# ArthurBrussee/brush

Measured on NVIDIA H100. Metric: fwd+bwd Mpix/s @1M Gaussians 1080p, higher is better.
Workload: dtype f32

## Files before the change

### brush_b200/csrc/bg_common.cuh

```cuda
#pragma once
#include <cuda_runtime.h>
#include <stdint.h>

#include "../../include/brush_b200.h"

namespace bg {

constexpr uint32_t TILE_W = 16;
constexpr uint32_t TILE_PIX = 256;
constexpr float ALPHA_CUTOFF_MID = 1.0f / 255.0f;
constexpr float ALPHA_CUTOFF_BAND = 1.0e-3f;

enum CtlOffsets : uint32_t {
    CTL_COUNTERS = 0,
    CTL_TICKETS = 16,
    CTL_HIST_DEPTH = 64,
    CTL_HIST_TILE = 64 + 1024,
    CTL_WORDS = 64 + 2048
};
enum TicketIds : uint32_t {
    TK_PROJECT = 0, TK_DEPTH_HIST = 1, TK_DEPTH_PASS0 = 2 , TK_SCAN = 6, TK_VISIBLE = 7,
    TK_TILE_HIST = 8, TK_TILE_PASS0 = 9 , TK_MISC = 13
};

constexpr uint32_t LB_INVALID = 0, LB_AGGREGATE = 1, LB_INCLUSIVE = 2;

__device__ __forceinline__ void lb_store(unsigned long long *p, uint32_t epoch, uint32_t status, uint32_t value) {
    unsigned long long w = ((unsigned long long)((epoch << 2) | status) << 32) | (unsigned long long)value;
    asm volatile("st.relaxed.gpu.global.u64 [%0], %1;" ::"l"(p), "l"(w) : "memory");
}
__device__ __forceinline__ unsigned long long lb_load(const unsigned long long *p) {
    unsigned long long w;
    asm volatile("ld.relaxed.gpu.global.u64 %0, [%1];" : "=l"(w) : "l"(p) : "memory");
    return w;
}
__device__ __forceinline__ uint32_t lb_status(unsigned long long w, uint32_t epoch) {
    uint32_t hi = (uint32_t)(w >> 32);
    return ((hi >> 2) == epoch) ? (hi & 3u) : LB_INVALID;
}
__device__ __forceinline__ uint32_t lb_value(unsigned long long w) { return (uint32_t)w; }

__device__ __forceinline__ uint32_t lb_lookback_warp(const unsigned long long *state, uint32_t tile, uint32_t epoch) {
    const uint32_t lane = threadIdx.x & 31u;
    uint32_t prefix = 0;
    int64_t pos = (int64_t)tile - 1;
    while (pos >= 0) {
        int64_t idx = pos - (int64_t)lane;
        uint32_t st, val;
        while (true) {
            st = LB_INCLUSIVE;
            val = 0;
            if (idx >= 0) {
                unsigned long long w = lb_load(state + idx);
                st = lb_status(w, epoch);
                val = lb_value(w);
            }
            if (__all_sync(0xffffffffu, st != LB_INVALID)) break;
        }
        uint32_t incl_mask = __ballot_sync(0xffffffffu, st == LB_INCLUSIVE);
        uint32_t first = incl_mask ? (uint32_t)(__ffs(incl_mask) - 1) : 32u;
        uint32_t contrib = (lane <= first) ? val : 0u;
        for (int o = 16; o > 0; o >>= 1) contrib += __shfl_xor_sync(0xffffffffu, contrib, o);
        prefix += contrib;
        if (incl_mask) break;
        pos -= 32;
    }
    return prefix;
}

__device__ __forceinline__ uint32_t smem_u32(const void *p) { return (uint32_t)__cvta_generic_to_shared(p); }
__device__ __forceinline__ void mbar_init(unsigned long long *bar, uint32_t count) {
    asm volatile("mbarrier.init.shared::cta.b64 [%0], %1;" ::"r"(smem_u32(bar)), "r"(count) : "memory");
    asm volatile("fence.mbarrier_init.release.cluster;" ::: "memory");
}
__device__ __forceinline__ void mbar_expect_tx(unsigned long long *bar, uint32_t bytes) {
    asm volatile("mbarrier.arrive.expect_tx.shared::cta.b64 _, [%0], %1;" ::"r"(smem_u32(bar)), "r"(bytes) : "memory");
}
__device__ __forceinline__ void tma_bulk_g2s(void *dst_smem, const void *src_gmem, uint32_t bytes, unsigned long long *bar) {
    asm volatile("cp.async.bulk.shared::cluster.global.mbarrier::complete_tx::bytes [%0], [%1], %2, [%3];" ::"r"(
                     smem_u32(dst_smem)),
                 "l"(src_gmem), "r"(bytes), "r"(smem_u32(bar))
                 : "memory");
}
__device__ __forceinline__ void mbar_wait(unsigned long long *bar, uint32_t parity) {
    asm volatile(
        "{\n"
        ".reg .pred p;\n"
        "WAIT_LOOP:\n"
        "mbarrier.try_wait.parity.shared::cta.b64 p, [%0], %1;\n"
        "@p bra WAIT_DONE;\n"
        "bra WAIT_LOOP;\n"
        "WAIT_DONE:\n"
        "}\n" ::"r"(smem_u32(bar)),
        "r"(parity)
        : "memory");
}

__device__ __forceinline__ float2 fadd2_rn(float2 a, float2 b) { return make_float2(__fadd_rn(a.x, b.x), __fadd_rn(a.y, b.y)); }
__device__ __forceinline__ float2 fmul2_rn(float2 a, float2 b) { return make_float2(__fmul_rn(a.x, b.x), __fmul_rn(a.y, b.y)); }
__device__ __forceinline__ float2 ffma2_rn(float2 a, float2 b, float2 c) {
    return make_float2(__fmaf_rn(a.x, b.x, c.x), __fmaf_rn(a.y, b.y, c.y));
}

__device__ __forceinline__ uint32_t block_exclusive_scan(uint32_t v, uint32_t *warp_sums, uint32_t *total) {
    const uint32_t lane = threadIdx.x & 31u, wid = threadIdx.x >> 5, nw = blockDim.x >> 5;
    uint32_t incl = v;
    for (int o = 1; o < 32; o <<= 1) {
        uint32_t t = __shfl_up_sync(0xffffffffu, incl, o);
        if (lane >= (uint32_t)o) incl += t;
    }
    if (lane == 31) warp_sums[wid] = incl;
    __syncthreads();
    if (wid == 0) {
        uint32_t s = (lane < nw) ? warp_sums[lane] : 0u;
        uint32_t si = s;
        for (int o = 1; o < 32; o <<= 1) {
            uint32_t t = __shfl_up_sync(0xffffffffu, si, o);
            if (lane >= (uint32_t)o) si += t;
        }
        if (lane < nw) warp_sums[lane] = si - s;
        if (lane == 31) warp_sums[32] = si;
    }
    __syncthreads();
    uint32_t r = warp_sums[wid] + incl - v;
    *total = warp_sums[32];
    __syncthreads();
    return r;
}

}
```

### brush_b200/csrc/blend_fwd.cu

```cuda
#include "blend_common.cuh"

namespace bg {

template <bool BWD_INFO, bool SMOOTH, bool DEPTH>
__global__ void __launch_bounds__(RASTER_THREADS)
blend_fwd_kernel(const float *__restrict__ projected, const uint32_t *__restrict__ cgid_from_isect,
                 uint32_t *__restrict__ tile_offsets, const uint32_t *__restrict__ gid_from_cgid,
                 float4 *__restrict__ out_f32, uint32_t *__restrict__ out_packed, float *__restrict__ visible,
                 uint32_t *__restrict__ live_masks, uint32_t *__restrict__ warp_batches, BlendUniforms u,
                 const float *__restrict__ depths, float *__restrict__ out_depth) {
    __shared__ BlendStage s_stage[RASTER_WARPS];
    __shared__ uint32_t s_max_useful;

    const uint32_t tile = blockIdx.x;
    const uint32_t tid = threadIdx.x, lane = tid & 31u, wid = tid >> 5;
    const uint32_t tile_x0 = (tile % u.tiles_x) * TILE_W, tile_y0 = (tile / u.tiles_x) * TILE_W;
    const uint32_t blk_x0 = tile_x0 + 8u * (wid & 1u), blk_y0 = tile_y0 + 8u * (wid >> 1);
    const uint32_t pix_x = blk_x0 + (lane & 7u), pix_y0 = blk_y0 + (lane >> 3), pix_y1 = pix_y0 + 4u;
    const bool inside0 = pix_x < u.img_w && pix_y0 < u.img_h;
    const bool inside1 = pix_x < u.img_w && pix_y1 < u.img_h;
    const float px = (float)pix_x + 0.5f, py0 = (float)pix_y0 + 0.5f;
    const float2 npy2 = make_float2(-py0, -(py0 + 4.0f));
    const float rx0 = (float)blk_x0 + 0.5f, rx1 = rx0 + 7.0f, ry0 = (float)blk_y0 + 0.5f, ry1 = ry0 + 7.0f;

    const uint32_t range_lo = tile_offsets[tile * 2], range_hi = tile_offsets[tile * 2 + 1];
    if (BWD_INFO && tid == 0) s_max_useful = range_lo;
    BlendStage &st = s_stage[wid];
    if (lane == 0) { mbar_init(&st.bar[0], 1); mbar_init(&st.bar[1], 1); }
    __syncthreads();
    uint32_t phase_bits = 0u;

    float2 T2 = make_float2(1.0f, 1.0f);
    float2 Tt2 = make_float2(inside0 ? 1.0f : 0.0f, inside1 ? 1.0f : 0.0f);
    float2 r2 = make_float2(0.0f, 0.0f), g2 = r2, b2 = r2, d2 = r2;
    uint32_t last_useful = range_lo;

    const uint32_t num_batches = (range_hi - range_lo + WB - 1) / WB;
    const size_t mbase = blend_mask_base(range_lo, tile) + wid;
    uint32_t batches_walked = 0;
    uint32_t next_id = 0;
    float next_z = 0.0f;
    auto prefetch = [&](uint32_t b) {
        const uint32_t start = range_lo + b * WB;
        const uint32_t count = min((uint32_t)WB, range_hi - start);
        const uint32_t id = lane < count ? __ldg(cgid_from_isect + start + lane) : 0u;
        next_id = id;
        if constexpr (DEPTH) next_z = lane < count ? __ldg(depths + id) : 0.0f;
        if (lane < count) st.ids[b & 1u][lane] = id;
        stage_rows_tma(st, b & 1u, count, projected, lane);
    };
    if (num_batches > 0 && __any_sync(0xffffffffu, inside0 || inside1)) {
        prefetch(0);
        for (uint32_t b = 0; b < num_batches; b++) {
            const uint32_t batch_start = range_lo + b * WB;
            const uint32_t count = min((uint32_t)WB, range_hi - batch_start);
            const uint32_t my_id = next_id;
            const float my_z = next_z;
            if (b + 1 < num_batches) prefetch(b + 1);
            mbar_wait(&st.bar[b & 1u], (phase_bits >> (b & 1u)) & 1u);
            phase_bits ^= 1u << (b & 1u);
            float *rows = st.rows[b & 1u];
            bool hit = false;
            if (lane < count) {
                float *mine = rows + lane * ROW;
                const float4 A = *reinterpret_cast<const float4 *>(mine);
                const float4 B = *reinterpret_cast<const float4 *>(mine + 4);
                const float bcol = mine[8];
                float pt = mine[ROW_PT];
                if constexpr (SMOOTH) pt += SMOOTH_THR_EXTRA;
                hit = block_may_hit(A.x, A.y, A.z, A.w, B.x, pt, rx0, rx1, ry0, ry1);
                *reinterpret_cast<float2 *>(mine + 6) = make_float2(fmaxf(B.z, 0.0f), fmaxf(B.w, 0.0f));
                mine[8] = fmaxf(bcol, 0.0f);
                if constexpr (DEPTH) mine[ROW_Z] = my_z;
            }
            uint32_t bits = __ballot_sync(0xffffffffu, hit);
            uint32_t used_m = 0, acted_m = 0;
            while (bits) {
                const uint32_t s = (uint32_t)__ffs(bits) - 1u;
                bits &= bits - 1u;
                const float *row = rows + s * ROW;
                const float4 A = *reinterpret_cast<const float4 *>(row);
                const float4 B = *reinterpret_cast<const float4 *>(row + 4);
                const float4 C = *reinterpret_cast<const float4 *>(row + 8);
                float2 dy2;
                const float2 sg = pair_sigma(A.x - px, A.y, C.y, C.z, C.w, npy2, dy2);
                const float2 gs = make_float2(ex2_approx(-sg.x), ex2_approx(-sg.y));
                const float2 oa = fmul2_rn(gs, bcast2(B.y));
                float a0 = fminf(0.999f, oa.x), a1 = fminf(0.999f, oa.y);
                bool act0, act1;
                if constexpr (SMOOTH) {
                    const float2 ae = smooth_alpha(make_float2(a0, a1), sg, act0, act1);
                    a0 = ae.x; a1 = ae.y;
                } else {
                    act0 = sg.x >= 0.0f && oa.x >= ALPHA_CUTOFF_MID; act1 = sg.y >= 0.0f && oa.y >= ALPHA_CUTOFF_MID;
                }
                const float2 nT = fmul2_rn(Tt2, fadd2_rn(make_float2(-a0, -a1), bcast2(1.0f)));
                const bool c0 = act0 && nT.x > 1.0e-4f, c1 = act1 && nT.y > 1.0e-4f;
                const float2 vis = fmul2_rn(make_float2(c0 ? a0 : 0.0f, c1 ? a1 : 0.0f), T2);
                r2 = ffma2_rn(bcast2(B.z), vis, r2);
                g2 = ffma2_rn(bcast2(B.w), vis, g2);
                b2 = ffma2_rn(bcast2(C.x), vis, b2);
                if constexpr (DEPTH) d2 = ffma2_rn(bcast2(row[ROW_Z]), vis, d2);
                const uint32_t bit = 1u << s;
                const bool acted = (Tt2.x > 1.0e-4f && act0) || (Tt2.y > 1.0e-4f && act1);
                if (c0 || c1) used_m |= bit;
                if (BWD_INFO && acted) acted_m |= bit;
                T2.x = c0 ? nT.x : T2.x;
                T2.y = c1 ? nT.y : T2.y;
                Tt2.x = act0 ? nT.x : Tt2.x;
                Tt2.y = act1 ? nT.y : Tt2.y;
            }
            const uint32_t used = __reduce_or_sync(0xffffffffu, used_m);
            if (BWD_INFO) {
                const uint32_t acted = __reduce_or_sync(0xffffffffu, acted_m);
                if (lane == 0) live_masks[mbase + (size_t)b * RASTER_WARPS] = acted;
                if ((used >> lane) & 1u) {
                    visible[__ldg(gid_from_cgid + my_id)] = 1.0f;
                    last_useful = batch_start + lane + 1;
                }
            }
            batches_walked = b + 1;
            if (__all_sync(0xffffffffu, !(Tt2.x > 1.0e-4f) && !(Tt2.y > 1.0e-4f))) {
                if (b + 1 < num_batches) mbar_wait(&st.bar[(b + 1) & 1u], (phase_bits >> ((b + 1) & 1u)) & 1u);
                break;
            }
            __syncwarp();
        }
    }

    auto write_pixel = [&](float T, float r, float g, float bl, float d, uint32_t pix_y) {
        const float fr = r + T * u.bg_r, fg = g + T * u.bg_g, fb = bl + T * u.bg_b, fa = 1.0f - T;
        const size_t pix_id = (size_t)pix_x + (size_t)pix_y * u.img_w;
        if (BWD_INFO) {
            out_f32[pix_id] = make_float4(fr, fg, fb, fa);
            if constexpr (DEPTH) out_depth[pix_id] = d;
        } else {
            uint32_t r8 = (uint32_t)fminf(fmaxf(fr * 255.0f, 0.0f), 255.0f);
            uint32_t g8 = (uint32_t)fminf(fmaxf(fg * 255.0f, 0.0f), 255.0f);
            uint32_t b8 = (uint32_t)fminf(fmaxf(fb * 255.0f, 0.0f), 255.0f);
            uint32_t a8 = (uint32_t)fminf(fmaxf(fa * 255.0f, 0.0f), 255.0f);
            out_packed[pix_id] = r8 | (g8 << 8) | (b8 << 16) | (a8 << 24);
        }
    };
    if (inside0) write_pixel(T2.x, r2.x, g2.x, b2.x, d2.x, pix_y0);
    if (inside1) write_pixel(T2.y, r2.y, g2.y, b2.y, d2.y, pix_y1);
    if (BWD_INFO) {
        if (lane == 0) warp_batches[tile * RASTER_WARPS + wid] = batches_walked;
        uint32_t m = last_useful;
        for (int o = 16; o > 0; o >>= 1) m = max(m, __shfl_xor_sync(0xffffffffu, m, o));
        __syncthreads();
        if (lane == 0 && m > range_lo) atomicMax(&s_max_useful, m);
        __syncthreads();
        if (tid == 0) tile_offsets[tile * 2 + 1] = s_max_useful;
    }
}

cudaError_t launch_blend_fwd(cudaStream_t s, bool bwd_info, bool smooth, uint32_t num_tiles, const float *projected,
                             const uint32_t *cgid_from_isect, uint32_t *tile_offsets, const uint32_t *gid_from_cgid, void *out_img,
                             float *visible, uint32_t *live_masks, uint32_t *warp_batches, uint32_t tiles_x, uint32_t w,
                             uint32_t h, const float *bg, const float *depths, float *out_depth) {
    BlendUniforms u;
    u.tiles_x = tiles_x; u.img_w = w; u.img_h = h; u.bg_r = bg[0]; u.bg_g = bg[1]; u.bg_b = bg[2];
#define BG_LAUNCH_FWD(B, S, D, F32, PACKED, LM, WBAT)                                                                    \
    blend_fwd_kernel<B, S, D><<<num_tiles, RASTER_THREADS, 0, s>>>(projected, cgid_from_isect, tile_offsets, gid_from_cgid, \
                                                                   F32, PACKED, visible, LM, WBAT, u, depths, out_depth)
    if (!bwd_info)
        BG_LAUNCH_FWD(false, false, false, nullptr, (uint32_t *)out_img, nullptr, nullptr);
    else if (out_depth && !smooth)
        BG_LAUNCH_FWD(true, false, true, (float4 *)out_img, nullptr, live_masks, warp_batches);
    else if (out_depth)
        BG_LAUNCH_FWD(true, true, true, (float4 *)out_img, nullptr, live_masks, warp_batches);
    else if (!smooth)
        BG_LAUNCH_FWD(true, false, false, (float4 *)out_img, nullptr, live_masks, warp_batches);
    else
        BG_LAUNCH_FWD(true, true, false, (float4 *)out_img, nullptr, live_masks, warp_batches);
#undef BG_LAUNCH_FWD
    return cudaGetLastError();
}

}
```

Before: 987.2.

## Use producer warp with shared 4-slot TMA ring for forward blend

New measurement: 1012 (median of 6 runs). 2.5% higher.

```diff
diff --git a/brush_b200/csrc/bg_common.cuh b/brush_b200/csrc/bg_common.cuh
--- a/brush_b200/csrc/bg_common.cuh
+++ b/brush_b200/csrc/bg_common.cuh
@@ -76,6 +76,9 @@
 __device__ __forceinline__ void mbar_expect_tx(unsigned long long *bar, uint32_t bytes) {
     asm volatile("mbarrier.arrive.expect_tx.shared::cta.b64 _, [%0], %1;" ::"r"(smem_u32(bar)), "r"(bytes) : "memory");
 }
+__device__ __forceinline__ void mbar_arrive(unsigned long long *bar) {
+    asm volatile("mbarrier.arrive.shared::cta.b64 _, [%0];" ::"r"(smem_u32(bar)) : "memory");
+}
 __device__ __forceinline__ void tma_bulk_g2s(void *dst_smem, const void *src_gmem, uint32_t bytes, unsigned long long *bar) {
     asm volatile("cp.async.bulk.shared::cluster.global.mbarrier::complete_tx::bytes [%0], [%1], %2, [%3];" ::"r"(
                      smem_u32(dst_smem)),
diff --git a/brush_b200/csrc/blend_fwd.cu b/brush_b200/csrc/blend_fwd.cu
--- a/brush_b200/csrc/blend_fwd.cu
+++ b/brush_b200/csrc/blend_fwd.cu
@@ -2,154 +2,178 @@
 
 namespace bg {
 
+constexpr int FWD_SLOTS = 4;
+constexpr int FWD_THREADS = RASTER_THREADS + 32;
+
+struct __align__(128) FwdSlot {
+    float rows[WB * ROW];
+    uint32_t ids[WB];
+    float z[WB];
+    uint32_t count;
+    unsigned long long full, empty;
+};
+
 template <bool BWD_INFO, bool SMOOTH, bool DEPTH>
-__global__ void __launch_bounds__(RASTER_THREADS)
+__global__ void __launch_bounds__(FWD_THREADS, 1)
 blend_fwd_kernel(const float *__restrict__ projected, const uint32_t *__restrict__ cgid_from_isect,
                  uint32_t *__restrict__ tile_offsets, const uint32_t *__restrict__ gid_from_cgid,
                  float4 *__restrict__ out_f32, uint32_t *__restrict__ out_packed, float *__restrict__ visible,
                  uint32_t *__restrict__ live_masks, uint32_t *__restrict__ warp_batches, BlendUniforms u,
                  const float *__restrict__ depths, float *__restrict__ out_depth) {
-    __shared__ BlendStage s_stage[RASTER_WARPS];
-    __shared__ uint32_t s_max_useful;
+    __shared__ FwdSlot s_slot[FWD_SLOTS];
+    __shared__ uint32_t s_max_useful, s_done;
 
     const uint32_t tile = blockIdx.x;
     const uint32_t tid = threadIdx.x, lane = tid & 31u, wid = tid >> 5;
-    const uint32_t tile_x0 = (tile % u.tiles_x) * TILE_W, tile_y0 = (tile / u.tiles_x) * TILE_W;
-    const uint32_t blk_x0 = tile_x0 + 8u * (wid & 1u), blk_y0 = tile_y0 + 8u * (wid >> 1);
-    const uint32_t pix_x = blk_x0 + (lane & 7u), pix_y0 = blk_y0 + (lane >> 3), pix_y1 = pix_y0 + 4u;
-    const bool inside0 = pix_x < u.img_w && pix_y0 < u.img_h;
-    const bool inside1 = pix_x < u.img_w && pix_y1 < u.img_h;
-    const float px = (float)pix_x + 0.5f, py0 = (float)pix_y0 + 0.5f;
-    const float2 npy2 = make_float2(-py0, -(py0 + 4.0f));
-    const float rx0 = (float)blk_x0 + 0.5f, rx1 = rx0 + 7.0f, ry0 = (float)blk_y0 + 0.5f, ry1 = ry0 + 7.0f;
-
     const uint32_t range_lo = tile_offsets[tile * 2], range_hi = tile_offsets[tile * 2 + 1];
-    if (BWD_INFO && tid == 0) s_max_useful = range_lo;
-    BlendStage &st = s_stage[wid];
-    if (lane == 0) { mbar_init(&st.bar[0], 1); mbar_init(&st.bar[1], 1); }
+    const uint32_t num_batches = (range_hi - range_lo + WB - 1) / WB;
+    if (tid == 0) { s_max_useful = range_lo; s_done = 0u; }
+    if (tid < FWD_SLOTS) { mbar_init(&s_slot[tid].full, 1); mbar_init(&s_slot[tid].empty, RASTER_WARPS); }
     __syncthreads();
-    uint32_t phase_bits = 0u;
-
-    float2 T2 = make_float2(1.0f, 1.0f);
-    float2 Tt2 = make_float2(inside0 ? 1.0f : 0.0f, inside1 ? 1.0f : 0.0f);
-    float2 r2 = make_float2(0.0f, 0.0f), g2 = r2, b2 = r2, d2 = r2;
-    uint32_t last_useful = range_lo;
-
-    const uint32_t num_batches = (range_hi - range_lo + WB - 1) / WB;
-    const size_t mbase = blend_mask_base(range_lo, tile) + wid;
-    uint32_t batches_walked = 0;
-    uint32_t next_id = 0;
-    float next_z = 0.0f;
-    auto prefetch = [&](uint32_t b) {
-        const uint32_t start = range_lo + b * WB;
-        const uint32_t count = min((uint32_t)WB, range_hi - start);
-        const uint32_t id = lane < count ? __ldg(cgid_from_isect + start + lane) : 0u;
-        next_id = id;
-        if constexpr (DEPTH) next_z = lane < count ? __ldg(depths + id) : 0.0f;
-        if (lane < count) st.ids[b & 1u][lane] = id;
-        stage_rows_tma(st, b & 1u, count, projected, lane);
-    };
-    if (num_batches > 0 && __any_sync(0xffffffffu, inside0 || inside1)) {
-        prefetch(0);
-        for (uint32_t b = 0; b < num_batches; b++) {
-            const uint32_t batch_start = range_lo + b * WB;
-            const uint32_t count = min((uint32_t)WB, range_hi - batch_start);
-            const uint32_t my_id = next_id;
-            const float my_z = next_z;
-            if (b + 1 < num_batches) prefetch(b + 1);
-            mbar_wait(&st.bar[b & 1u], (phase_bits >> (b & 1u)) & 1u);
-            phase_bits ^= 1u << (b & 1u);
-            float *rows = st.rows[b & 1u];
-            bool hit = false;
+
+    if (wid == RASTER_WARPS) {
+        auto load_ids = [&](uint32_t b) {
+            const uint32_t start = range_lo + b * WB;
+            return lane < min((uint32_t)WB, range_hi - start) ? __ldg(cgid_from_isect + start + lane) : 0u;
+        };
+        uint32_t b = 0;
+        uint32_t next_id = num_batches > 0 ? load_ids(0) : 0u;
+        for (; b < num_batches; b++) {
+            if (*reinterpret_cast<volatile uint32_t *>(&s_done) == (uint32_t)RASTER_WARPS) break;
+            const uint32_t id = next_id;
+            if (b + 1 < num_batches) next_id = load_ids(b + 1);
+            FwdSlot &sl = s_slot[b % FWD_SLOTS];
+            if (b >= FWD_SLOTS) mbar_wait(&sl.empty, ((b / FWD_SLOTS) & 1u) ^ 1u);
+            const uint32_t count = min((uint32_t)WB, range_hi - (range_lo + b * WB));
             if (lane < count) {
-                float *mine = rows + lane * ROW;
-                const float4 A = *reinterpret_cast<const float4 *>(mine);
-                const float4 B = *reinterpret_cast<const float4 *>(mine + 4);
-                const float bcol = mine[8];
-                float pt = mine[ROW_PT];
-                if constexpr (SMOOTH) pt += SMOOTH_THR_EXTRA;
-                hit = block_may_hit(A.x, A.y, A.z, A.w, B.x, pt, rx0, rx1, ry0, ry1);
-                *reinterpret_cast<float2 *>(mine + 6) = make_float2(fmaxf(B.z, 0.0f), fmaxf(B.w, 0.0f));
-                mine[8] = fmaxf(bcol, 0.0f);
-                if constexpr (DEPTH) mine[ROW_Z] = my_z;
-            }
-            uint32_t bits = __ballot_sync(0xffffffffu, hit);
-            uint32_t used_m = 0, acted_m = 0;
-            while (bits) {
-                const uint32_t s = (uint32_t)__ffs(bits) - 1u;
-                bits &= bits - 1u;
-                const float *row = rows + s * ROW;
-                const float4 A = *reinterpret_cast<const float4 *>(row);
-                const float4 B = *reinterpret_cast<const float4 *>(row + 4);
-                const float4 C = *reinterpret_cast<const float4 *>(row + 8);
-                float2 dy2;
-                const float2 sg = pair_sigma(A.x - px, A.y, C.y, C.z, C.w, npy2, dy2);
-                const float2 gs = make_float2(ex2_approx(-sg.x), ex2_approx(-sg.y));
-                const float2 oa = fmul2_rn(gs, bcast2(B.y));
-                float a0 = fminf(0.999f, oa.x), a1 = fminf(0.999f, oa.y);
-                bool act0, act1;
-                if constexpr (SMOOTH) {
-                    const float2 ae = smooth_alpha(make_float2(a0, a1), sg, act0, act1);
-                    a0 = ae.x; a1 = ae.y;
-                } else {
-                    act0 = sg.x >= 0.0f && oa.x >= ALPHA_CUTOFF_MID; act1 = sg.y >= 0.0f && oa.y >= ALPHA_CUTOFF_MID;
-                }
-                const float2 nT = fmul2_rn(Tt2, fadd2_rn(make_float2(-a0, -a1), bcast2(1.0f)));
-                const bool c0 = act0 && nT.x > 1.0e-4f, c1 = act1 && nT.y > 1.0e-4f;
-                const float2 vis = fmul2_rn(make_float2(c0 ? a0 : 0.0f, c1 ? a1 : 0.0f), T2);
-                r2 = ffma2_rn(bcast2(B.z), vis, r2);
-                g2 = ffma2_rn(bcast2(B.w), vis, g2);
-                b2 = ffma2_rn(bcast2(C.x), vis, b2);
-                if constexpr (DEPTH) d2 = ffma2_rn(bcast2(row[ROW_Z]), vis, d2);
-                const uint32_t bit = 1u << s;
-                const bool acted = (Tt2.x > 1.0e-4f && act0) || (Tt2.y > 1.0e-4f && act1);
-                if (c0 || c1) used_m |= bit;
-                if (BWD_INFO && acted) acted_m |= bit;
-                T2.x = c0 ? nT.x : T2.x;
-                T2.y = c1 ? nT.y : T2.y;
-                Tt2.x = act0 ? nT.x : Tt2.x;
-                Tt2.y = act1 ? nT.y : Tt2.y;
-            }
-            const uint32_t used = __reduce_or_sync(0xffffffffu, used_m);
+                sl.ids[lane] = id;
+                if constexpr (DEPTH) sl.z[lane] = __ldg(depths + id);
+            }
+            __syncwarp();
+            if (lane == 0) {
+                sl.count = count;
+                mbar_expect_tx(&sl.full, count * (ROW * 4u));
+                for (uint32_t r = 0; r < count; r++)
+                    tma_bulk_g2s(&sl.rows[r * ROW], projected + (size_t)sl.ids[r] * ROW, ROW * 4u, &sl.full);
+            }
+        }
+        FwdSlot &sl = s_slot[b % FWD_SLOTS];
+        if (b >= FWD_SLOTS) mbar_wait(&sl.empty, ((b / FWD_SLOTS) & 1u) ^ 1u);
+        if (lane == 0) { sl.count = 0u; mbar_arrive(&sl.full); }
+    } else {
+        const uint32_t tile_x0 = (tile % u.tiles_x) * TILE_W, tile_y0 = (tile / u.tiles_x) * TILE_W;
+        const uint32_t blk_x0 = tile_x0 + 8u * (wid & 1u), blk_y0 = tile_y0 + 8u * (wid >> 1);
+        const uint32_t pix_x = blk_x0 + (lane & 7u), pix_y0 = blk_y0 + (lane >> 3), pix_y1 = pix_y0 + 4u;
+        const bool inside0 = pix_x < u.img_w && pix_y0 < u.img_h;
+        const bool inside1 = pix_x < u.img_w && pix_y1 < u.img_h;
+        const float px = (float)pix_x + 0.5f, py0 = (float)pix_y0 + 0.5f;
+        const float2 npy2 = make_float2(-py0, -(py0 + 4.0f));
+        const float rx0 = (float)blk_x0 + 0.5f, rx1 = rx0 + 7.0f, ry0 = (float)blk_y0 + 0.5f, ry1 = ry0 + 7.0f;
+
+        float2 T2 = make_float2(1.0f, 1.0f);
+        float2 Tt2 = make_float2(inside0 ? 1.0f : 0.0f, inside1 ? 1.0f : 0.0f);
+        float2 r2 = make_float2(0.0f, 0.0f), g2 = r2, b2 = r2, d2 = r2;
+        uint32_t last_useful = range_lo;
+        const size_t mbase = blend_mask_base(range_lo, tile) + wid;
+        uint32_t batches_walked = 0;
+        bool blending = __any_sync(0xffffffffu, inside0 || inside1);
+        if (!blending && lane == 0) atomicAdd(&s_done, 1u);
+        for (uint32_t b = 0;; b++) {
+            FwdSlot &sl = s_slot[b % FWD_SLOTS];
+            mbar_wait(&sl.full, (b / FWD_SLOTS) & 1u);
+            const uint32_t count = sl.count;
+            if (count == 0) break;
+            if (blending) {
+                const uint32_t batch_start = range_lo + b * WB;
+                const float *rows = sl.rows;
+                bool hit = false;
+                if (lane < count) {
+                    const float *mine = rows + lane * ROW;
+                    const float4 A = *reinterpret_cast<const float4 *>(mine);
+                    float pt = mine[ROW_PT];
+                    if constexpr (SMOOTH) pt += SMOOTH_THR_EXTRA;
+                    hit = block_may_hit(A.x, A.y, A.z, A.w, mine[4], pt, rx0, rx1, ry0, ry1);
+                }
+                uint32_t bits = __ballot_sync(0xffffffffu, hit);
+                uint32_t used_m = 0, acted_m = 0;
+                while (bits) {
+                    const uint32_t s = (uint32_t)__ffs(bits) - 1u;
+                    bits &= bits - 1u;
+                    const float *row = rows + s * ROW;
+                    const float4 A = *reinterpret_cast<const float4 *>(row);
+                    const float4 B = *reinterpret_cast<const float4 *>(row + 4);
+                    const float4 C = *reinterpret_cast<const float4 *>(row + 8);
+                    float2 dy2;
+                    const float2 sg = pair_sigma(A.x - px, A.y, C.y, C.z, C.w, npy2, dy2);
+                    const float2 gs = make_float2(ex2_approx(-sg.x), ex2_approx(-sg.y));
+                    const float2 oa = fmul2_rn(gs, bcast2(B.y));
+                    float a0 = fminf(0.999f, oa.x), a1 = fminf(0.999f, oa.y);
+                    bool act0, act1;
+                    if constexpr (SMOOTH) {
+                        const float2 ae = smooth_alpha(make_float2(a0, a1), sg, act0, act1);
+                        a0 = ae.x; a1 = ae.y;
+                    } else {
+                        act0 = sg.x >= 0.0f && oa.x >= ALPHA_CUTOFF_MID; act1 = sg.y >= 0.0f && oa.y >= ALPHA_CUTOFF_MID;
+                    }
+                    const float2 nT = fmul2_rn(Tt2, fadd2_rn(make_float2(-a0, -a1), bcast2(1.0f)));
+                    const bool c0 = act0 && nT.x > 1.0e-4f, c1 = act1 && nT.y > 1.0e-4f;
+                    const float2 vis = fmul2_rn(make_float2(c0 ? a0 : 0.0f, c1 ? a1 : 0.0f), T2);
+                    r2 = ffma2_rn(bcast2(fmaxf(B.z, 0.0f)), vis, r2);
+                    g2 = ffma2_rn(bcast2(fmaxf(B.w, 0.0f)), vis, g2);
+                    b2 = ffma2_rn(bcast2(fmaxf(C.x, 0.0f)), vis, b2);
+                    if constexpr (DEPTH) d2 = ffma2_rn(bcast2(sl.z[s]), vis, d2);
+                    const uint32_t bit = 1u << s;
+                    const bool acted = (Tt2.x > 1.0e-4f && act0) || (Tt2.y > 1.0e-4f && act1);
+                    if (c0 || c1) used_m |= bit;
+                    if (BWD_INFO && acted) acted_m |= bit;
+                    T2.x = c0 ? nT.x : T2.x;
+                    T2.y = c1 ? nT.y : T2.y;
+                    Tt2.x = act0 ? nT.x : Tt2.x;
+                    Tt2.y = act1 ? nT.y : Tt2.y;
+                }
+                const uint32_t used = __reduce_or_sync(0xffffffffu, used_m);
+                if (BWD_INFO) {
+                    const uint32_t acted = __reduce_or_sync(0xffffffffu, acted_m);
+                    if (lane == 0) live_masks[mbase + (size_t)b * RASTER_WARPS] = acted;
+                    if ((used >> lane) & 1u) {
+                        visible[__ldg(gid_from_cgid + sl.ids[lane])] = 1.0f;
+                        last_useful = batch_start + lane + 1;
+                    }
+                }
+                batches_walked = b + 1;
+                if (__all_sync(0xffffffffu, !(Tt2.x > 1.0e-4f) && !(Tt2.y > 1.0e-4f))) {
+                    blending = false;
+                    if (lane == 0) atomicAdd(&s_done, 1u);
+                }
+            }
+            __syncwarp();
+            if (lane == 0) mbar_arrive(&sl.empty);
+        }
+
+        auto write_pixel = [&](float T, float r, float g, float bl, float d, uint32_t pix_y) {
+            const float fr = r + T * u.bg_r, fg = g + T * u.bg_g, fb = bl + T * u.bg_b, fa = 1.0f - T;
+            const size_t pix_id = (size_t)pix_x + (size_t)pix_y * u.img_w;
             if (BWD_INFO) {
-                const uint32_t acted = __reduce_or_sync(0xffffffffu, acted_m);
-                if (lane == 0) live_masks[mbase + (size_t)b * RASTER_WARPS] = acted;
-                if ((used >> lane) & 1u) {
-                    visible[__ldg(gid_from_cgid + my_id)] = 1.0f;
-                    last_useful = batch_start + lane + 1;
-                }
-            }
-            batches_walked = b + 1;
-            if (__all_sync(0xffffffffu, !(Tt2.x > 1.0e-4f) && !(Tt2.y > 1.0e-4f))) {
-                if (b + 1 < num_batches) mbar_wait(&st.bar[(b + 1) & 1u], (phase_bits >> ((b + 1) & 1u)) & 1u);
-                break;
-            }
-            __syncwarp();
+                out_f32[pix_id] = make_float4(fr, fg, fb, fa);
+                if constexpr (DEPTH) out_depth[pix_id] = d;
+            } else {
+                uint32_t r8 = (uint32_t)fminf(fmaxf(fr * 255.0f, 0.0f), 255.0f);
+                uint32_t g8 = (uint32_t)fminf(fmaxf(fg * 255.0f, 0.0f), 255.0f);
+                uint32_t b8 = (uint32_t)fminf(fmaxf(fb * 255.0f, 0.0f), 255.0f);
+                uint32_t a8 = (uint32_t)fminf(fmaxf(fa * 255.0f, 0.0f), 255.0f);
+                out_packed[pix_id] = r8 | (g8 << 8) | (b8 << 16) | (a8 << 24);
+            }
+        };
+        if (inside0) write_pixel(T2.x, r2.x, g2.x, b2.x, d2.x, pix_y0);
+        if (inside1) write_pixel(T2.y, r2.y, g2.y, b2.y, d2.y, pix_y1);
+        if (BWD_INFO) {
+            if (lane == 0) warp_batches[tile * RASTER_WARPS + wid] = batches_walked;
+            uint32_t m = last_useful;
+            for (int o = 16; o > 0; o >>= 1) m = max(m, __shfl_xor_sync(0xffffffffu, m, o));
+            if (lane == 0 && m > range_lo) atomicMax(&s_max_useful, m);
         }
     }
-
-    auto write_pixel = [&](float T, float r, float g, float bl, float d, uint32_t pix_y) {
-        const float fr = r + T * u.bg_r, fg = g + T * u.bg_g, fb = bl + T * u.bg_b, fa = 1.0f - T;
-        const size_t pix_id = (size_t)pix_x + (size_t)pix_y * u.img_w;
-        if (BWD_INFO) {
-            out_f32[pix_id] = make_float4(fr, fg, fb, fa);
-            if constexpr (DEPTH) out_depth[pix_id] = d;
-        } else {
-            uint32_t r8 = (uint32_t)fminf(fmaxf(fr * 255.0f, 0.0f), 255.0f);
-            uint32_t g8 = (uint32_t)fminf(fmaxf(fg * 255.0f, 0.0f), 255.0f);
-            uint32_t b8 = (uint32_t)fminf(fmaxf(fb * 255.0f, 0.0f), 255.0f);
-            uint32_t a8 = (uint32_t)fminf(fmaxf(fa * 255.0f, 0.0f), 255.0f);
-            out_packed[pix_id] = r8 | (g8 << 8) | (b8 << 16) | (a8 << 24);
-        }
-    };
-    if (inside0) write_pixel(T2.x, r2.x, g2.x, b2.x, d2.x, pix_y0);
-    if (inside1) write_pixel(T2.y, r2.y, g2.y, b2.y, d2.y, pix_y1);
     if (BWD_INFO) {
-        if (lane == 0) warp_batches[tile * RASTER_WARPS + wid] = batches_walked;
-        uint32_t m = last_useful;
-        for (int o = 16; o > 0; o >>= 1) m = max(m, __shfl_xor_sync(0xffffffffu, m, o));
-        __syncthreads();
-        if (lane == 0 && m > range_lo) atomicMax(&s_max_useful, m);
         __syncthreads();
         if (tid == 0) tile_offsets[tile * 2 + 1] = s_max_useful;
     }
@@ -162,8 +186,8 @@
     BlendUniforms u;
     u.tiles_x = tiles_x; u.img_w = w; u.img_h = h; u.bg_r = bg[0]; u.bg_g = bg[1]; u.bg_b = bg[2];
 #define BG_LAUNCH_FWD(B, S, D, F32, PACKED, LM, WBAT)                                                                    \
-    blend_fwd_kernel<B, S, D><<<num_tiles, RASTER_THREADS, 0, s>>>(projected, cgid_from_isect, tile_offsets, gid_from_cgid, \
-                                                                   F32, PACKED, visible, LM, WBAT, u, depths, out_depth)
+    blend_fwd_kernel<B, S, D><<<num_tiles, FWD_THREADS, 0, s>>>(projected, cgid_from_isect, tile_offsets, gid_from_cgid, \
+                                                                F32, PACKED, visible, LM, WBAT, u, depths, out_depth)
     if (!bwd_info)
         BG_LAUNCH_FWD(false, false, false, nullptr, (uint32_t *)out_img, nullptr, nullptr);
     else if (out_depth && !smooth)
```
